# zengxianyu/sketchedit

Hardware: AMD Instinct MI355X
Metric: images/sec (higher is better)
Workload: dtype f32; 1 GPU; SketchEdit inference forward (netM+netG, use_cam, pool max) 256x256 batch 32 per GPU, procedural weights; global_batch=32, size=256, per_gpu_batch=32, execution=default, two streams

## Files before the change

sketchedit_amd/csrc/se_api.hip:

```cpp
#include "../../include/sketchedit_hip.h"
#include "../../include/sketchedit_png.h"
#include "../../include/sketchedit_jpg.h"
#include "../../include/sketchedit_jpg2.h"
#include "../../include/sketchedit_feather.h"
#include "../../include/sketchedit_fill.h"
#include "../../include/sketchedit_select.h"
#include "../../include/sketchedit_lasso.h"
#include "../../include/sketchedit_outline.h"
#include "se_kernels.h"
#include "se_pack.h"

#include <cstdarg>
#include <cstdint>
#include <cstdlib>
#include <cstdio>
#include <cstring>
#include <algorithm>
#include <map>
#include <mutex>
#include <numeric>
#include <string>
#include <vector>

using namespace se;
// ... 280 lines not shown
  p.src = src0; p.wpk = wimg; p.bias = L.d_b; p.dst = dst;
  p.B = B; p.Hin = Hin; p.Win = Win; p.C = C0; p.CG = CG; p.T = L.T; p.KW = KW;
  p.magicCG = (65536 + CG - 1) / CG; p.magicKW = 256 / KW + 1;
  for (int gi = 0; gi < nch * 8 + 8; ++gi)
    if (((gi * p.magicCG) >> 16) != gi / CG) return 0;
  for (int t = 0; t <= L.T + 8; ++t)
    if (((t * p.magicKW) >> 8) != t / KW) return 0;
  p.pad = pad; p.up2 = d.up ? 1 : 0; p.OH = Ho; p.OW = Wo;
  p.G = bf ? (L.G + 7) & ~7 : L.G;
  p.nch = nch; p.NP = L.NP;
  udiv_magic_host((unsigned)(C0 * es / 16), &p.div_cg_m, &p.div_cg_l);
  udiv_magic_host((unsigned)p.RW, &p.div_rw_m, &p.div_rw_l);
  p.ty = (Hin + TR - 1) / TR; p.tx = (Win + 15) / 16;
  p.act = d.act; p.bf16 = bf ? 1 : 0; p.xcd = xcd_remap_enabled();
  {
    const double alg = 2.0 * (double)B * Ho * Wo * d.cout * d.cin * d.k * d.k;
    const double exec = 2.0 * (double)B * Hin * Win * (d.up ? 4.0 : 1.0) * L.NP * (nch * (bf ? 64.0 : 32.0));
    set_launch_cost(alg, (double)es * ((double)B * Hin * Win * d.cin + (double)B * Ho * Wo * (d.cout / 2)), d.name, exec);
  }
  HIPCHK(c, launch_rtile(p, c->st));
  *done = true;
  return 0;
}

int run_gather(se_ctx* c, const Layer& L, bool bf, const float* src0, int C0, const float* src1, int C1, int src1_vec, float* dst,
               int B, int Hin, int Win, int Ho, int Wo, int pad) {
  const LayerDef& d = L.def;
  const DirectImage& di = L.direct[bf];
  const int es = bf ? 2 : 4, gran = bf ? 8 : 4;
  GConvParams p;
  memset(&p, 0, sizeof p);
  p.bf16 = bf ? 1 : 0;
  p.src0 = src0; p.src1 = src1 ? src1 : src0; p.wpk = di.w; p.bias = L.d_b; p.dst = dst; p.zeros = c->zeros;
  p.B = B; p.Hin = Hin; p.Win = Win; p.Ho = d.up ? Hin : Ho; p.Wo = d.up ? Win : Wo;
  p.up2 = d.up ? 1 : 0; p.OH = Ho; p.OW = Wo;
  p.C0 = C0; p.C1 = C1 ? C1 : C0; p.C0g = C0 / gran; p.CG = di.CG;
  const int KW = d.up ? 2 : d.k;
  p.T = L.T; p.KW = KW; p.stride = d.stride; p.dil = d.rate; p.pad = pad;
  p.magicCG = (65536 + di.CG - 1) / di.CG; p.magicKW = 256 / KW + 1; p.magicKH = L.T / KW;
  for (int gi = 0; gi < di.nch * 8 + 8; ++gi)
    if (((gi * p.magicCG) >> 16) != gi / di.CG) return fail(c, "layer %s: magic division check failed", d.name);
  for (int t = 0; t <= L.T + 8; ++t)
    if (((t * p.magicKW) >> 8) != t / KW) return fail(c, "layer %s: magic tap division check failed", d.name);
  const int Gs = bf ? (L.G + 7) & ~7 : L.G;
  if ((double)B * Hin * Win * (C0 > C1 ? C0 : C1) * es >= 2147483648.0 || (double)B * Ho * Wo * Gs * es >= 2147483648.0)
    return fail(c, "layer %s: a tensor of this launch exceeds 2^31 bytes (32-bit byte offsets) -- split the batch", d.name);
  for (int j = 0; j < p.magicKH; ++j) p.rep |= 1u << (j * KW);
  udiv_magic_host((unsigned)(p.Ho * p.Wo), &p.div_hw_m, &p.div_hw_l);
  udiv_magic_host((unsigned)p.Wo, &p.div_w_m, &p.div_w_l);
  p.Hlim = Hin; p.Wlim = Win;
  p.src1_vec = src1_vec; p.nch = di.nch; p.G = Gs; p.act = d.act; p.total_pix = B * p.Ho * p.Wo;
  p.xcd = xcd_remap_enabled();
  p.np_full = L.NP; p.nf_full = L.NP / 32; p.small_grid = c->low_latency ? 1 : 0;
  {
    const double alg = 2.0 * (double)B * Ho * Wo * d.cout * d.cin * d.k * d.k;
    const double exec = 2.0 * (double)B * p.Ho * p.Wo * (d.up ? 4.0 : 1.0) * L.NP * (di.nch * (bf ? 64.0 : 32.0));
    set_launch_cost(alg, (double)es * ((double)B * Hin * Win * d.cin + (double)B * Ho * Wo * (d.cout / 2)), d.name, exec);
  }
  HIPCHK(c, launch_gconv(L.cfg, p, c->st));
  return 0;
}

static bool rconv16_dual_ok(const Layer& L, const LayerDef& d, int Hin, int Win) {
  if (opt(OPT_RCONV16_DUAL) == 0) return false;
  return L.d_w16s && (d.rate % 2) == 0 && Win / d.rate == 8 && Hin / d.rate <= 8 && Hin / d.rate >= 4;
}

int run_gconv16(se_ctx* c, const Layer& L, const float* src0, int C0, const float* src1, int C1, int src1_vec, float* dst,
                int B, int Hin, int Win, int Ho, int Wo, int pad) {
  const LayerDef& d = L.def;
  if (!L.direct[1].w) return fail(c, "layer %s: no bf16 weight image", d.name);
  if ((C0 + C1) != L.direct[1].CG * 8) return fail(c, "layer %s: bf16 source channels %d+%d != packed %d", d.name, C0, C1, L.direct[1].CG * 8);
  const bool use_rconv = opt(OPT_RCONV16) != 0;
  {
    if (opt(OPT_VECBIAS) != 0 && use_rconv && !c->low_latency && src1 && src1_vec && c->vbias_ws && c->vec32 && L.d_w16s && L.d_wv16 &&
        d.k == 3 && d.stride == 1 && d.rate == 1 && !d.up && d.cin == 192 && d.cout == 192 && C0 == 96 && C1 == 96 &&
        Hin >= 12 && Win >= 12 && (long long)B * Hin * Win * 192 < (1ll << 31)) {
      HIPCHK(c, launch_vecbias(L.d_wv16, c->vec32, c->vbias_ws, B, 96, c->st, 1));
      RConvParams rp;
      memset(&rp, 0, sizeof rp);
      rp.src = src0; rp.wpk = L.d_w16s; rp.bias = L.d_b; rp.dst = dst; rp.vbias = c->vbias_ws;
      rp.B = B; rp.h = Hin; rp.w = Win; rp.d = 1; rp.hs = Hin; rp.ws = Win;
      rp.ty = (Hin + 7) / 8; rp.tx = (Win + 15) / 16;
      rp.act = d.act; rp.xcd = xcd_remap_enabled();
      const double alg = 2.0 * (double)B * Ho * Wo * d.cout * d.cin * 9;
      set_launch_cost(alg, 2.0 * 2.0 * (double)B * Hin * Win * 96, d.name, 2.0 * (double)B * Hin * Win * 192.0 * 864.0);
      HIPCHK(c, launch_rconv16(rp, c->st));
      return 0;
    }
  }
  if (use_rconv && !c->low_latency && d.k == 3 && d.stride == 1 && !d.up && d.cin == 96 && d.cout == 192 && !src1 && C0 == 96 &&
      (Hin % d.rate) == 0 && (Win % d.rate) == 0 && L.direct[1].nch == 14 && L.d_w16s && (long long)B * Hin * Win * 192 < (1ll << 31) &&
      ((Hin / d.rate >= 12 && Win / d.rate >= 12) || rconv16_dual_ok(L, d, Hin, Win))) {
    RConvParams rp;
    memset(&rp, 0, sizeof rp);
    rp.dual = !(Hin / d.rate >= 12 && Win / d.rate >= 12);
    rp.src = src0; rp.wpk = L.d_w16s; rp.bias = L.d_b; rp.dst = dst;
    rp.B = B; rp.h = Hin; rp.w = Win; rp.d = d.rate; rp.hs = Hin / d.rate; rp.ws = Win / d.rate;
    rp.ty = (rp.hs + 7) / 8; rp.tx = (rp.ws + 15) / 16;
    rp.act = d.act; rp.xcd = xcd_remap_enabled();
    const double alg = 2.0 * (double)B * Ho * Wo * d.cout * d.cin * 9;
    set_launch_cost(alg, 2.0 * 2.0 * (double)B * Hin * Win * 96, d.name, 2.0 * (double)B * Hin * Win * 192.0 * 864.0);
    HIPCHK(c, launch_rconv16(rp, c->st));
    return 0;
  }
  const bool use_rconv96 = opt(OPT_RCONV96) != 0;
// ... 2525 lines not shown
```

sketchedit_amd/csrc/se_attention.hip:

```cpp
#include "se_device.h"

#include <cstdlib>

namespace se {


template <bool BF16>
__global__ void att2_prep_kernel(const AttParams p) {
  const long idx = (long)blockIdx.x * 256 + threadIdx.x;
  const long nx = (long)p.B * p.h * p.w * (BF16 ? 12 : 24);
  if (idx < nx) {
    if (BF16) {
      const int cg = idx % 12;
      const long pix = idx / 12;
      const int b = pix / (p.h * p.w);
      const uint4 v = *(const uint4*)((const char*)p.x + idx * 16);
      const f32x4 r0 = *(const f32x4*)(p.rn + b * 96 + cg * 8), r1 = *(const f32x4*)(p.rn + b * 96 + cg * 8 + 4);
      *(uint4*)((char*)p.xn + idx * 16) =
          make_uint4(pack_bf16x2(bf16_lo(v.x) * r0[0], bf16_hi(v.x) * r0[1]), pack_bf16x2(bf16_lo(v.y) * r0[2], bf16_hi(v.y) * r0[3]),
                     pack_bf16x2(bf16_lo(v.z) * r1[0], bf16_hi(v.z) * r1[1]), pack_bf16x2(bf16_lo(v.w) * r1[2], bf16_hi(v.w) * r1[3]));
    } else {
      const int cg = idx % 24;
      const long pix = idx / 24;
      const int b = pix / (p.h * p.w);
// ... 98 lines not shown
#pragma unroll
    for (int o = 32; o > 0; o >>= 1) { a += __shfl_xor(a, o); bb += __shfl_xor(bb, o); g += __shfl_xor(g, o); }
    bb -= g;
  }
  if (lane == 0) { p.ea[gi] = a; p.eb[gi] = bb; }
}
__global__ __launch_bounds__(256) void att2_eoff4_kernel(const AttParams p) {
  const long gi = (long)blockIdx.x * 256 + threadIdx.x;
  if (gi >= (long)p.B * p.Rp) return;
  const int b = (int)(gi / p.Rp), k = (int)(gi - (long)b * p.Rp);
  const float* ea = p.ea + (size_t)b * p.Rp, *eb = p.eb + (size_t)b * p.Rp;
  auto at = [&](const float* t, int i) { return i < p.R ? t[i] : 0.f; };
  p.ea4[gi] = ((at(ea, k) + at(ea, k + 1)) + at(ea, k + p.wc)) + at(ea, k + p.wc + 1);
  const float b4 = ((at(eb, k) + at(eb, k + 1)) + at(eb, k + p.wc)) + at(eb, k + p.wc + 1);
  p.kadd2[gi] = fmaf(b4, p.kmul[gi], p.kadd[gi]);
}

template <int NT, int PT, bool BF16>
__global__ __launch_bounds__(256) void att2_pair_kernel(const AttParams p) {
  constexpr int PXB = BF16 ? 192 : 384;
  constexpr int PIX = PT * 64, NP = NT * 16;
  constexpr int XBYTES = PIX * 128, WBYTES = NP * 128;
  constexpr int NX = PT * 2, NW = (NT * 2 + 3) / 4;
  extern __shared__ __attribute__((aligned(16))) char smem[];
  char* Xb = smem;
  char* Wb = smem + 2 * XBYTES;

  const int tid = threadIdx.x, lane = tid & 63;
  const int w = __builtin_amdgcn_readfirstlane(tid >> 6);
  int b = blockIdx.z, bx = blockIdx.x, by = blockIdx.y;
  if (p.sym) {
    static_assert(PIX == 4 * NP, "tile enumeration");
    const int lb = xcd_tile(blockIdx.x, gridDim.x);
    b = lb / p.symT;
    const int t = lb - b * p.symT;
    int pn = (int)((sqrtf(64.f + 128.f * (float)t) - 8.f) * (1.f / 64.f));
    while (32 * (pn + 1) * (pn + 1) + 8 * (pn + 1) <= t) ++pn;
    while (32 * pn * pn + 8 * pn > t) --pn;
    const int u = t - (32 * pn * pn + 8 * pn);
    if (u < 64 * pn) {
      bx = u >> 4;
      by = 16 * pn + (u & 15);
    } else {
      const int v = u - 64 * pn;
      const int j = v < 16 ? 0 : (v < 28 ? 1 : (v < 36 ? 2 : 3));
      bx = 4 * pn + j;
      by = 16 * pn + 4 * j + (v - (j == 0 ? 0 : (j == 1 ? 16 : (j == 2 ? 28 : 36))));
    }
    if (by * NP >= p.R) return;
  }
  const int q0 = bx * PIX, k0 = by * NP;
  auto origin = [&](int i) -> unsigned {
    if (i >= p.R) return 0x80000000u;
    const int ry = i / p.wc, rx = i - ry * p.wc;
    return (unsigned)(((2 * ry) * p.w + 2 * rx) * PXB);
  };
  const se_i32x4 rs_q = make_rsrc((const char*)(p.sym ? p.xn : p.x) + (size_t)b * p.h * p.w * PXB, (unsigned)p.h * p.w * (unsigned)PXB);
  const se_i32x4 rs_k = make_rsrc((const char*)p.xn + (size_t)b * p.h * p.w * PXB, (unsigned)p.h * p.w * (unsigned)PXB);
  unsigned qo[NX], ko[NW];
#pragma unroll
  for (int i = 0; i < NX; ++i) qo[i] = origin(q0 + (i * 4 + w) * 8 + (lane >> 3));
#pragma unroll
  for (int j = 0; j < NW; ++j) ko[j] = (j * 4 + w) < NT * 2 ? origin(k0 + (j * 4 + w) * 8 + (lane >> 3)) : 0x80000000u;

  const int s_log = (lane & 7) ^ (4 * (w & 1) + (lane >> 4));
  int off0, off1;
  frag_offsets(lane, off0, off1);
  const unsigned lds_x = lds_addr_of(Xb), lds_w = lds_addr_of(Wb);

  auto stage = [&](int ch, int buf) {
    const int gi = ch * 8 + s_log;
    constexpr int GPP = BF16 ? 12 : 24;
    const int tap = (gi * (BF16 ? 5462 : 2731)) >> 16, cg = gi - tap * GPP;
    const unsigned doff = (unsigned)((__mul24(tap >> 1, p.w) + (tap & 1)) * PXB + cg * 16);
    const unsigned xdst = lds_x + buf * XBYTES, wdst = lds_w + buf * WBYTES;
#pragma unroll
    for (int i = 0; i < NX; ++i) bufdma16(qo[i] + doff, rs_q, xdst + (i * 4 + w) * 1024);
#pragma unroll
    for (int j = 0; j < NW; ++j) {
      const int rbk = j * 4 + w;
      if (rbk < NT * 2) bufdma16(ko[j] + doff, rs_k, wdst + rbk * 1024);
    }
  };

  f32x4 acc[NT][PT];
#pragma unroll
  for (int nt = 0; nt < NT; ++nt)
#pragma unroll
    for (int pt = 0; pt < PT; ++pt) acc[nt][pt] = (f32x4){0.f, 0.f, 0.f, 0.f};
  if (BF16 && p.e16) {
    const float* ea = p.ea + (size_t)b * p.Rp, *eb = p.eb + (size_t)b * p.Rp;
    float eq[PT];
#pragma unroll
    for (int pt = 0; pt < PT; ++pt) eq[pt] = ea[min(q0 + w * PT * 16 + pt * 16 + (lane & 15), p.Rp - 1)];
#pragma unroll
    for (int nt = 0; nt < NT; ++nt) {
      const f32x4 ek = *(const f32x4*)(eb + min(k0 + nt * 16 + (lane >> 4) * 4, p.Rp - 4));
#pragma unroll
      for (int pt = 0; pt < PT; ++pt) acc[nt][pt] = (f32x4){-(eq[pt] + ek[0]), -(eq[pt] + ek[1]), -(eq[pt] + ek[2]), -(eq[pt] + ek[3])};
    }
  }
  constexpr int NCH = BF16 ? 6 : 12;
  stage(0, 0);
  dma_wait_all();
  __syncthreads();
  for (int ch = 0; ch < NCH; ++ch) {
    const int buf = ch & 1;
    if (ch + 1 < NCH) stage(ch + 1, buf ^ 1);
    if (BF16) mfma_chunk16<NT, PT>(acc, Wb + buf * WBYTES, Xb + buf * XBYTES + w * PT * 2048, off0, off1);
    else mfma_chunk<NT, PT>(acc, Wb + buf * WBYTES, Xb + buf * XBYTES + w * PT * 2048, off0, off1);
    dma_wait_all();
    __syncthreads();
  }
  constexpr int TS = NT * 16 + 4;
  static_assert(4 * PT * 16 * TS * 4 <= 2 * XBYTES + 2 * WBYTES, "transpose buffer exceeds the staging buffers");
  float* T = (float*)smem + w * (PT * 16 * TS);
  const int q = lane >> 4;
#pragma unroll
  for (int nt = 0; nt < NT; ++nt)
#pragma unroll
    for (int pt = 0; pt < PT; ++pt) *(f32x4*)(T + (pt * 16 + (lane & 15)) * TS + nt * 16 + q * 4) = acc[nt][pt];
  constexpr int PPR = NT * 4;
  constexpr int RPI = 64 / PPR;
  const int pc = lane % PPR, pr = lane / PPR;
  const int j = k0 + pc * 4;
#pragma unroll
  for (int rr = 0; rr < PT * 16; rr += RPI) {
    const int row = rr + pr;
    const f32x4 v = *(const f32x4*)(T + row * TS + pc * 4);
    const int i = q0 + w * PT * 16 + row;
    if (i < p.R && j < p.Rp) {
      if (BF16 && p.e16) {
        typedef _Float16 h4 __attribute__((ext_vector_type(4)));
        typedef unsigned u32x2 __attribute__((ext_vector_type(2)));
        auto sat = [](float t) { return __builtin_amdgcn_fmed3f(t, -65504.f, 65504.f); };
        const h4 hv = (h4){(_Float16)sat(v[0]), (_Float16)sat(v[1]), (_Float16)sat(v[2]), (_Float16)sat(v[3])};
        __builtin_nontemporal_store(__builtin_bit_cast(u32x2, hv), (u32x2*)((char*)p.E + (((size_t)b * p.R + i) * p.Rp + j) * 2));
      } else __builtin_nontemporal_store(v, (f32x4*)(p.E + ((size_t)b * p.R + i) * p.Rp + j));
    }
  }
  if (!BF16 && p.sym && k0 >= q0 + PIX) {
    constexpr int PPM = PT * 4;
    constexpr int RPM = 64 / PPM;
    const int mc = lane % PPM, mr = lane / PPM;
    const int qcol = q0 + w * PT * 16 + mc * 4;
#pragma unroll
    for (int kk0 = 0; kk0 < NT * 16; kk0 += RPM) {
      const int kk = kk0 + mr;
      const float* t = T + (mc * 4) * TS + kk;
      const f32x4 v = (f32x4){t[0], t[TS], t[2 * TS], t[3 * TS]};
      const int srow = k0 + kk;
      if (srow < p.R && qcol < p.Rp) __builtin_nontemporal_store(v, (f32x4*)(p.E + ((size_t)b * p.R + srow) * p.Rp + qcol));
    }
  }
}

DEVFN bool tile_order(long q, int B, int ny, int nx, int& b, int& y, int& x) {
  const int ty = (ny + 7) >> 3, tx = (nx + 7) >> 3;
  const long per = (long)ty * tx * 64;
  b = (int)(q / per);
  const int rem = (int)(q - (long)b * per), t = rem >> 6, in = rem & 63;
  y = (t / tx) * 8 + (in >> 3);
  x = (t % tx) * 8 + (in & 7);
  return b < B && y < ny && x < nx;
}
static inline long tile_order_count(int B, int ny, int nx) { return (long)B * ((ny + 7) >> 3) * ((nx + 7) >> 3) * 64; }

template <bool BF16>
__global__ __launch_bounds__(256) void att2_softmax_kernel(const AttParams p) {
  const int lane = threadIdx.x & 63;
  int b, iy, ix;
  if (!tile_order((long)xcd_tile(blockIdx.x, gridDim.x) * 4 + (threadIdx.x >> 6), p.B, p.hs, p.ws, b, iy, ix)) return;
  const int r0 = iy * p.wc + ix;
  const float* E0 = p.E + ((size_t)b * p.R + r0) * p.Rp;
  const float* E1 = E0 + p.Rp;
  const float* E2 = E0 + (size_t)p.wc * p.Rp;
  const float* E3 = E2 + p.Rp;
  const float* vr = p.validR + (size_t)b * p.Rp;
  float* P = p.P + ((size_t)b * p.R + r0) * p.Rp;
  unsigned short* P16 = (unsigned short*)p.P + ((size_t)b * p.R + r0) * p.Rp;
  const int o2 = p.wc, o3 = p.wc + 1;
  auto score = [&](int s, float v) { return (E0[s] + E1[s + 1] + E2[s + o2] + E3[s + o3]) * v * p.scale; };
  float m = -INFINITY;
  for (int s = lane; s < p.R; s += 64) {
    const float v = vr[s];
    if (v >= 0.f) {
      const float sc = score(s, v);
      if (!BF16) P[s] = sc;
      m = fmaxf(m, sc);
    }
  }
#pragma unroll
  for (int o = 32; o > 0; o >>= 1) m = fmaxf(m, __shfl_xor(m, o));
  float sum = 0.f;
  for (int s = lane; s < p.R; s += 64) {
    const float v = vr[s];
    if (v >= 0.f) {
      const float e = expf((BF16 ? score(s, v) : P[s]) - m);
      if (!BF16) P[s] = e;
      sum += e;
    }
  }
#pragma unroll
// ... 662 lines not shown
#pragma unroll
  for (int pt = 0; pt < PT; ++pt) {
    const int i = t0 + (w * PT + pt) * 16 + (lane & 15);
    if (i >= p.R) continue;
    const int yy = i / p.wc, xx = i - yy * p.wc;
    char* o = (char*)p.out + (((long)(b * p.h + 2 * yy + py) * p.w + 2 * xx + px) * 96 + rh * NP) * ES;
#pragma unroll
    for (int nt = 0; nt < NT; ++nt) {
      const f32x4 a = acc[nt][pt];
      if (BF16) *(uint2*)(o + (nt * 16 + q * 4) * 2) = make_uint2(pack_bf16x2(a[0], a[1]), pack_bf16x2(a[2], a[3]));
      else *(f32x4*)(o + (nt * 16 + q * 4) * 4) = a;
    }
  }
}

template <bool BF16>
__global__ void att2_similar_kernel(const AttParams p) {
  const long idx = (long)blockIdx.x * 256 + threadIdx.x;
  if (idx >= (long)p.B * p.L * p.L) return;
  const int i = idx % p.L;
  const long bj = idx / p.L;
  const int j = bj % p.L, b = bj / p.L;
  const int r = (i / p.ws) * p.wc + i % p.ws, s = (j / p.ws) * p.wc + j % p.ws;
  const size_t at = ((size_t)b * p.R + r) * p.Rp + s;
  p.similar[idx] = BF16 ? bf16_lo(((const unsigned short*)p.P)[at]) : p.P[at];
}

static bool att_lds_form(int wc) {
  return wc % 4 == 0 && wc <= 124 && opt(OPT_ATT_PTILDE_LDS) != 0;
}
static bool att_fused(bool bf16, int Rp, int wc) {
  const int e1 = opt(OPT_ATT_FUSED), e2 = opt(OPT_ATT_FUSED_BF16);
  const int f32mode = e1 < 0 ? -1 : (e1 != 0 ? 1 : 0);
  if (bf16) {
    if (e2 == 0) return false;
    if (e2 > 0) return f32mode < 0 ? att_lds_form(wc) : f32mode == 1;
    return f32mode != 0 && att_lds_form(wc);
  }
  return f32mode < 0 ? (Rp <= 1024 || att_lds_form(wc)) : f32mode == 1;
}

template <bool BF16>
static void enqueue_att2_prep(const AttParams& p, hipStream_t st) {
  const long n = (long)p.B * p.h * p.w * (BF16 ? 12 : 24);
  hipLaunchKernelGGL(att2_prep_kernel<BF16>, dim3((unsigned)((n + 255) / 256)), dim3(256), 0, st, p);
  hipLaunchKernelGGL(att2_transpose_kernel<BF16>, dim3(p.Rp / 32, 4, p.B), dim3(256), 0, st, p);
}

template <bool BF16>
static hipError_t launch_attention_v2_t(const AttParams& p0, hipStream_t st) {
  AttParams p = p0;
  const bool fused = att_fused(BF16, p.Rp, p.wc) && !p.similar && p.stats;
  p.Pt = fused ? p.P : p.E;
  p.sym = (!BF16 && opt(OPT_ATT_SYM) != 0) ? 1 : 0;
  const bool stats_lds = opt(OPT_ATT_STATS_LDS) != 0;
  p.e16 = (BF16 && fused && att_lds_form(p.wc) && stats_lds && opt(OPT_ATT_E16) != 0) ? 1 : 0;
  {
    const long n = (long)p.B * p.h * p.w * (BF16 ? 12 : 24);
    if (p.guard < p.wc + 8 || ((n + 255) / 256) * 256 < (long)p.guard) return hipErrorInvalidValue;
    ProfScope ps_(st, PL_ATT_PREP);
    enqueue_att2_prep<BF16>(p, st);
    if (p.e16) {
      const long nr = (long)p.B * p.Rp;
      hipLaunchKernelGGL(att2_emean1_kernel<BF16>, dim3(p.hc, p.B), dim3(384), 0, st, p);
      hipLaunchKernelGGL(att2_emean2_kernel, dim3(p.B), dim3(384), 0, st, p);
      hipLaunchKernelGGL(att2_eoff_kernel<BF16>, dim3((unsigned)((nr + 3) / 4)), dim3(256), 0, st, p);
      hipLaunchKernelGGL(att2_eoff4_kernel, dim3((unsigned)((nr + 255) / 256)), dim3(256), 0, st, p);
    }
  }
  {
    const double alg_flops = 2.0 * p.B * (double)p.L * p.L * 1536.0;
    const double alg_bytes = (BF16 ? 2.0 : 4.0) * 2.0 * p.B * (double)p.h * p.w * 96;
    const long big_grid = (long)((p.R + 255) / 256) * ((p.R + 63) / 64) * p.B;
    if (big_grid >= 512) {
      constexpr int NT = 4, PT = 4;
      constexpr int LDS = 2 * PT * 64 * 128 + 2 * NT * 16 * 128;
      hipError_t e = ensure_max_lds((const void*)att2_pair_kernel<NT, PT, BF16>, LDS);
      if (e != hipSuccess) return e;
      dim3 grid((p.R + PT * 64 - 1) / (PT * 64), (p.Rp + NT * 16 - 1) / (NT * 16), p.B);
      if (p.sym) {
        const int np = ((int)grid.y + 15) / 16;
        p.symT = 32 * np * np + 8 * np;
        grid = dim3((unsigned)(p.symT * p.B));
      }
      set_launch_cost(alg_flops, alg_bytes, nullptr, 2.0 * (double)grid.x * grid.y * grid.z * (PT * 64.0) * (NT * 16.0) * 384.0);
      set_launch_grid((long)grid.x * grid.y * grid.z);
      ProfScope ps_(st, PL_ATT_SCORE, p.sym ? "att_pair_sym" : "att_pair_all");
      hipLaunchKernelGGL((att2_pair_kernel<NT, PT, BF16>), grid, dim3(256), LDS, st, p);
    } else {
      constexpr int NT = 2, PT = 2;
      constexpr int LDS = 2 * PT * 64 * 128 + 2 * NT * 16 * 128;
      hipError_t e = ensure_max_lds((const void*)att2_pair_kernel<NT, PT, BF16>, LDS);
      if (e != hipSuccess) return e;
      dim3 grid((p.R + PT * 64 - 1) / (PT * 64), (p.Rp + NT * 16 - 1) / (NT * 16), p.B);
      if (p.sym) {
        const int np = ((int)grid.y + 15) / 16;
        p.symT = 32 * np * np + 8 * np;
        grid = dim3((unsigned)(p.symT * p.B));
      }
      set_launch_cost(alg_flops, alg_bytes, nullptr, 2.0 * (double)grid.x * grid.y * grid.z * (PT * 64.0) * (NT * 16.0) * 384.0);
      set_launch_grid((long)grid.x * grid.y * grid.z);
      ProfScope ps_(st, PL_ATT_SCORE, p.sym ? "att_pair_sym" : "att_pair_all");
      hipLaunchKernelGGL((att2_pair_kernel<NT, PT, BF16>), grid, dim3(256), LDS, st, p);
    }
  }
  if (fused) {
// ... 109 lines not shown
```

sketchedit_amd/csrc/se_device.h:

```cpp
#pragma once
#include "se_kernels.h"

namespace se {

typedef float f32x4 __attribute__((ext_vector_type(4)));
typedef float f32x2 __attribute__((ext_vector_type(2)));
#define DEVFN __device__ __forceinline__

DEVFN void glds16(const void* gsrc, unsigned lds_addr) {
  unsigned keep;
  asm volatile(
      "s_mov_b32 %0, m0\n\t"
      "s_mov_b32 m0, %2\n\t"
      "s_nop 0\n\t"
      "global_load_lds_dwordx4 %1, off\n\t"
      "s_mov_b32 m0, %0"
      : "=&s"(keep)
      : "v"(gsrc), "s"(lds_addr)
      : "memory");
}
DEVFN void glds16_s(const void* sbase, unsigned voff, unsigned lds_addr) {
  unsigned keep;
  asm volatile(
      "s_mov_b32 %0, m0\n\t"
// ... 33 lines not shown
      "s_mov_b32 m0, %3\n\t"
      "s_nop 0\n\t"
      "buffer_load_dword %1, %2, 0 offen lds\n\t"
      "s_mov_b32 m0, %0"
      : "=&s"(keep)
      : "v"(voff), "s"(rsrc), "s"(lds_addr)
      : "memory");
}
DEVFN void dma_wait_all() { asm volatile("s_waitcnt vmcnt(0)" ::: "memory"); }

DEVFN unsigned lds_addr_of(const void* p) {
  return (unsigned)(size_t)(const __attribute__((address_space(3))) char*)p;
}

DEVFN float sigmoidf_(float x) { return 1.f / (1.f + expf(-x)); }
DEVFN float fast_exp(float x) { return __expf(x); }
DEVFN float fast_rcp(float x) { return __builtin_amdgcn_rcpf(x); }
DEVFN float elu_fast(float x) {
  const float e = __builtin_amdgcn_exp2f(fminf(x, 0.f) * 1.44269504088896340736f) - 1.f;
  return x > 0.f ? x : e;
}
DEVFN float sigmoid_fast(float x) { return fast_rcp(1.f + fast_exp(-x)); }
DEVFN float act_fast(float x, float eluw) {
  const float n = __builtin_amdgcn_fmed3f(x * 1.44269504088896340736f, -__builtin_inff(), 0.f);
  const float neg = fmaf(__builtin_amdgcn_exp2f(n), eluw, -eluw);
  return __builtin_amdgcn_fmed3f(x, neg, __builtin_inff());
}
DEVFN float tanh_fast(float x) { return 1.f - 2.f * fast_rcp(1.f + fast_exp(2.f * x)); }

DEVFN unsigned udiv_magic(unsigned x, unsigned m, int l) {
  const unsigned t = __umulhi(m, x);
  return (t + ((x - t) >> (l < 1 ? l : 1))) >> (l > 1 ? l - 1 : 0);
}

DEVFN int xcd_tile(int bid, int nblocks) {
  const int q = nblocks >> 3, r = nblocks & 7;
  const int xcd = bid & 7, idx = bid >> 3;
  return (xcd < r ? xcd * (q + 1) : r * (q + 1) + (xcd - r) * q) + idx;
}

DEVFN bool class_tile(int bid, int ntiles, int xcd_remap, int& tile, int& cls) {
  const int xcd = bid & 7, g = bid >> 3;
  cls = g & 3;
  const int b2 = ((g >> 2) << 3) | xcd;
  if (b2 >= ntiles) return false;
  tile = xcd_remap ? xcd_tile(b2, ntiles) : b2;
  return true;
}
static inline int class_tile_grid(int ntiles) { return 4 * ((ntiles + 7) & ~7); }

struct NoHook { DEVFN void operator()(int) const {} };
template <int NT, int PT, typename Hook = NoHook>
DEVFN void mfma_chunk(f32x4 (&acc)[NT][PT], const char* __restrict__ Wt, const char* __restrict__ Xt, int off0,
                      int off1, Hook hook = Hook()) {
  f32x4 xb[2][PT];
#pragma unroll
  for (int half = 0; half < 2; ++half)
#pragma unroll
    for (int pt = 0; pt < PT; ++pt) xb[half][pt] = *(const f32x4*)(Xt + pt * 2048 + (half ? off1 : off0));
  f32x4 wn = *(const f32x4*)(Wt + off0);
#pragma unroll
  for (int half = 0; half < 2; ++half) {
#pragma unroll
    for (int nt = 0; nt < NT; ++nt) {
      const f32x4 wa = wn;
      if (nt + 1 < NT) wn = *(const f32x4*)(Wt + (nt + 1) * 2048 + (half ? off1 : off0));
      else if (half == 0) wn = *(const f32x4*)(Wt + off1);
#pragma unroll
      for (int r = 0; r < 4; ++r) {
#pragma unroll
        for (int pt = 0; pt < PT; ++pt)
          acc[nt][pt] = __builtin_amdgcn_mfma_f32_16x16x4f32(wa[r], xb[half][pt][r], acc[nt][pt], 0, 0, 0);
      }
      hook(half * NT + nt);
    }
  }
}

typedef __bf16 bf16x8 __attribute__((ext_vector_type(8)));
DEVFN unsigned pack_bf16x2(float lo, float hi) {
  unsigned r;
  asm("v_cvt_pk_bf16_f32 %0, %1, %2" : "=v"(r) : "v"(lo), "v"(hi));
  return r;
}
DEVFN float bf16_lo(unsigned u) { return __uint_as_float(u << 16); }
DEVFN float bf16_hi(unsigned u) { return __uint_as_float(u & 0xffff0000u); }

template <int NT, int PT, typename Hook = NoHook>
DEVFN void mfma_chunk16(f32x4 (&acc)[NT][PT], const char* __restrict__ Wt, const char* __restrict__ Xt, int off0,
                        int off1, Hook hook = Hook()) {
  constexpr int NU = 2 * NT, DEPTH = NU < 6 ? NU : 6;
  bf16x8 xb[2][PT];
#pragma unroll
  for (int half = 0; half < 2; ++half)
#pragma unroll
    for (int pt = 0; pt < PT; ++pt) xb[half][pt] = *(const bf16x8*)(Xt + pt * 2048 + (half ? off1 : off0));
  bf16x8 wq[DEPTH];
#pragma unroll
  for (int u = 0; u < DEPTH; ++u) wq[u] = *(const bf16x8*)(Wt + (u % NT) * 2048 + (u / NT ? off1 : off0));
  __builtin_amdgcn_sched_barrier(0);
#pragma unroll
  for (int u = 0; u < NU; ++u) {
    const int half = u / NT, nt = u % NT;
    const bf16x8 wa = wq[u % DEPTH];
    if (u + DEPTH < NU) wq[u % DEPTH] = *(const bf16x8*)(Wt + ((u + DEPTH) % NT) * 2048 + ((u + DEPTH) / NT ? off1 : off0));
    __builtin_amdgcn_sched_barrier(0);
#pragma unroll
    for (int pt = 0; pt < PT; ++pt)
      acc[nt][pt] = __builtin_amdgcn_mfma_f32_16x16x32_bf16(wa, xb[half][pt], acc[nt][pt], 0, 0, 0);
    hook(u);
    __builtin_amdgcn_sched_barrier(0);
  }
}

DEVFN void frag_offsets(int lane, int& off0, int& off1) {
  const int swz = (lane >> 1) & 7;
  off0 = (lane & 15) * 128 + (((lane >> 4) ^ swz) << 4);
  off1 = (lane & 15) * 128 + (((4 + (lane >> 4)) ^ swz) << 4);
}

DEVFN unsigned load_dword_within(const unsigned char* p, const unsigned char* lo, const unsigned char* hi) {
  if (p >= lo && p + 4 <= hi) return *(const unsigned*)p;
  unsigned v = 0;
#pragma unroll
  for (int i = 0; i < 4; ++i)
    if (p + i >= lo && p + i < hi) v |= (unsigned)p[i] << (8 * i);
  return v;
}
DEVFN unsigned load4_within(const unsigned char* a, const unsigned char* lo, const unsigned char* hi) {
  const unsigned char* a0 = (const unsigned char*)((size_t)a & ~(size_t)3);
  const int sh = (int)((size_t)a & 3) * 8;
  const unsigned d0 = load_dword_within(a0, lo, hi);
  if (!sh) return d0;
  return (d0 >> sh) | (load_dword_within(a0 + 4, lo, hi) << (32 - sh));
}
DEVFN unsigned clear_locked(unsigned sel, unsigned lk) {
#pragma unroll
  for (int p = 0; p < 4; ++p)
    if ((lk >> (8 * p)) & 255u) sel &= ~(255u << (8 * p));
  return sel;
}

struct ProfScope {
  hipStream_t st;
  int idx = -1;
  ProfScope(hipStream_t s, int label, const char* form = nullptr);
  ~ProfScope();
};

}
```

sketchedit_amd/csrc/se_gconv.hip:

```cpp
#include "se_device.h"

#include <cstdlib>

namespace se {

template <int NT, int PT, bool MIXED, int WPS, bool FAST, bool SPLIT, bool BF16>
__global__ __launch_bounds__(256, WPS) void gconv_kernel(const GConvParams p) {
  constexpr int PIX = PT * 64;
  constexpr int NP = NT * 16;
  constexpr int ES = BF16 ? 2 : 4;
  constexpr int XBYTES = PIX * 128, WBYTES = NP * 128;
  constexpr int NX = PT * 2;
  extern __shared__ __attribute__((aligned(16))) char smem[];
  char* Xb = smem;
  char* Wb = smem + 2 * XBYTES;
  int2* rowtab = (int2*)smem;

  const int tid = threadIdx.x, lane = tid & 63;
  const float eluw = p.act == 0 ? 1.f : 0.f;
  const int w = __builtin_amdgcn_readfirstlane(tid >> 6);
  int tile_idx = p.xcd ? xcd_tile(blockIdx.x, gridDim.x) : (int)blockIdx.x, cls = 0;
  if (p.up2 && !class_tile((int)blockIdx.x, (p.total_pix + PIX - 1) / PIX, p.xcd, tile_idx, cls)) return;
  const int tile_base = tile_idx * PIX;
  const int py = cls >> 1, px = cls & 1;
// ... 82 lines not shown
    fast_head(ch);
#pragma unroll
    for (int q = 0; q < NPIECE; ++q) fast_piece(ch, buf, q);
  };
  auto stage_any = [&](int ch, int buf) {
    const int gi = ch * 8 + s_log;
    const int tap = (gi * p.magicCG) >> 16, cg = gi - tap * p.CG;
    const int ky = (tap * p.magicKW) >> 8, kx = tap - ky * p.KW;
    const int dy = ky * p.dil - pady, dx = kx * p.dil - padx;
    const bool tapok = tap < p.T;
    const bool first = cg < p.C0g;
    const char* base = (const char*)(first ? p.src0 : p.src1);
    const int cs = (first ? p.C0 : p.C1) * ES;
    const int coff = (first ? cg : cg - p.C0g) * 16;
    const bool vec = (!first) && p.src1_vec;
    const unsigned xdst = lds_x + buf * XBYTES;
#pragma unroll
    for (int i = 0; i < NX; ++i) {
      int iy = (ryx[i] >> 16) + dy, ix = (ryx[i] & 0xffff) + dx;
      const bool ok = tapok & ((unsigned)iy < (unsigned)p.Hlim) & ((unsigned)ix < (unsigned)p.Wlim);
      iy >>= p.ushift;
      ix >>= p.ushift;
      const unsigned pix = vec ? (unsigned)rb[i] : (unsigned)((rb[i] * p.Hin + iy) * p.Win + ix);
      const char* g = base + (size_t)pix * (unsigned)cs + (unsigned)coff;
      g = ok ? g : (const char*)p.zeros;
      glds16(g, xdst + (i * 4 + w) * 1024);
    }
    const unsigned wdst = lds_w + buf * WBYTES;
    const float* wsrc = wbase + (size_t)ch * npf * 32 + lane * 4;
#pragma unroll
    for (int j = 0; j < (NT * 2 + 3) / 4; ++j) {
      const int rbk = j * 4 + w;
      if (rbk < NT * 2) glds16(wsrc + full_rbk(rbk) * 256, wdst + rbk * 1024);
    }
  };
  auto stage = [&](int ch, int buf) {
    if (FAST) stage_fast(ch, buf);
    else stage_any(ch, buf);
  };

  f32x4 acc[NT][PT];
#pragma unroll
  for (int nt = 0; nt < NT; ++nt)
#pragma unroll
    for (int pt = 0; pt < PT; ++pt) acc[nt][pt] = (f32x4){0.f, 0.f, 0.f, 0.f};

  stage(0, 0);
  dma_wait_all();
  __syncthreads();
  for (int ch = 0; ch < p.nch; ++ch) {
    const int buf = ch & 1;
    if (FAST) {
      const bool more = ch + 1 < p.nch;
      if (more) fast_head(ch + 1);
      constexpr int SLOTS = NT, PER = (NPIECE + SLOTS - 1) / SLOTS;
      auto hook = [&](int slot) {
        if (more) {
#pragma unroll
          for (int u = 0; u < PER; ++u) fast_piece(ch + 1, buf ^ 1, slot * PER + u);
        }
      };
      if (BF16) mfma_chunk16<NT, PT>(acc, Wb + buf * WBYTES, Xb + buf * XBYTES + w * PT * 2048, off0, off1, hook);
      else mfma_chunk<NT, PT>(acc, Wb + buf * WBYTES, Xb + buf * XBYTES + w * PT * 2048, off0, off1, hook);
    } else {
      if (ch + 1 < p.nch) stage(ch + 1, buf ^ 1);
      if (BF16) mfma_chunk16<NT, PT>(acc, Wb + buf * WBYTES, Xb + buf * XBYTES + w * PT * 2048, off0, off1);
      else mfma_chunk<NT, PT>(acc, Wb + buf * WBYTES, Xb + buf * XBYTES + w * PT * 2048, off0, off1);
    }
    dma_wait_all();
    __syncthreads();
  }

  const int q = lane >> 4;
  auto out_off = [&](int pidx) -> size_t {
    if (!p.up2) return (size_t)pidx * p.G;
    const int b = (int)udiv_magic((unsigned)pidx, p.div_hw_m, p.div_hw_l), rem = pidx - b * HoWo;
    const int yy = (int)udiv_magic((unsigned)rem, p.div_w_m, p.div_w_l), xx = rem - yy * p.Wo;
    return ((size_t)(b * p.OH + 2 * yy + py) * p.OW + 2 * xx + px) * p.G;
  };
  if (!MIXED) {
    constexpr int NF = NT / 2;
    const int nff = SPLIT ? p.nf_full : NF;
#pragma unroll
    for (int nt = 0; nt < NF; ++nt) {
      const int c0 = (grp * NF + nt) * 16 + q * 4;
      const f32x4 bf = *(const f32x4*)(p.bias + c0);
      const f32x4 bg = *(const f32x4*)(p.bias + nff * 16 + c0);
#pragma unroll
      for (int pt = 0; pt < PT; ++pt) {
        const int pidx = tile_base + (w * PT + pt) * 16 + (lane & 15);
        f32x4 o;
#pragma unroll
        for (int r = 0; r < 4; ++r) {
          const float f = acc[nt][pt][r] + bf[r];
          const float g = acc[nt + NF][pt][r] + bg[r];
          const float a = act_fast(f, eluw);
          o[r] = a * sigmoid_fast(g);
        }
        if (c0 < p.G && pidx < p.total_pix) {
          if (BF16) *(uint2*)((char*)p.dst + (out_off(pidx) + c0) * 2) = make_uint2(pack_bf16x2(o[0], o[1]), pack_bf16x2(o[2], o[3]));
          else *(f32x4*)(p.dst + out_off(pidx) + c0) = o;
        }
      }
    }
  } else {
#pragma unroll
    for (int nt = 0; nt < NT; ++nt) {
      const int c0 = (grp * NT + nt) * 8 + (q & 1) * 4 + (q >> 1) * 2;
      const f32x4 bq = *(const f32x4*)(p.bias + (grp * NT + nt) * 16 + q * 4);
#pragma unroll
      for (int pt = 0; pt < PT; ++pt) {
        const int pidx = tile_base + (w * PT + pt) * 16 + (lane & 15);
        const f32x4 v = acc[nt][pt] + bq;
        const auto s02 = __builtin_amdgcn_permlane32_swap(__float_as_uint(v[0]), __float_as_uint(v[2]), false, false);
        const auto s13 = __builtin_amdgcn_permlane32_swap(__float_as_uint(v[1]), __float_as_uint(v[3]), false, false);
        const float f0 = __uint_as_float(s02[0]), g0 = __uint_as_float(s02[1]);
        const float f1 = __uint_as_float(s13[0]), g1 = __uint_as_float(s13[1]);
        float2 o;
        o.x = act_fast(f0, eluw) * sigmoid_fast(g0);
        o.y = act_fast(f1, eluw) * sigmoid_fast(g1);
// ... 72 lines not shown
```

sketchedit_amd/csrc/se_kernels.h:

```cpp
#pragma once
#include <hip/hip_runtime.h>
#include <stddef.h>
#include <stdint.h>

#include <vector>

struct se_window;

namespace se {

enum ProfLabel { PL_GCONV_N192 = 0, PL_GCONV_N96, PL_GCONV_N48, PL_GCONV_N24, PL_WINO_N192, PL_WINO_N96, PL_WINO_UP96, PL_SMALL_CONV, PL_PACK, PL_COLREDUCE,
                 PL_ATT_PREP, PL_ATT_SCORE, PL_ATT_SOFTMAX, PL_ATT_BOXSUM, PL_ATT_PV, PL_LAYOUT,
                 PL_ATT_STREAM_STATS, PL_ATT_STREAM_OUT, PL_RESIZE_H, PL_RESIZE_V, PL_WINDOW_GATHER, PL_WINDOW_BORDER, PL_WINDOW_PASTE,
                 PL_WINDOW_RESAMPLE_H, PL_WINDOW_PASTE_V, PL_WINDOW_SAVE, PL_WINDOW_SWAP, PL_WINDOW_LOCK_GATHER, PL_WINDOW_PASTE_LOCKED,
                 PL_WINDOW_PASTE_V_LOCKED, PL_SKETCH_TILES, PL_SKETCH_STROKES, PL_PNG_ROWS, PL_PNG_STRIPES,
                 PL_PNG_FINISH, PL_JPG_BLOCKS, PL_JPG_ROWS, PL_JPG_FINISH, PL_JPG2_BLOCKS, PL_JPG2_HIST, PL_JPG2_TABLES,
                 PL_WINDOW_PASTE_FEATHER, PL_FILL_MASKS, PL_FILL_KEEP, PL_SELECT_SIMILAR, PL_SELECT_FLOOD, PL_SELECT_GROW,
                 PL_LASSO_FILL, PL_PLANE_COMBINE, PL_OUTLINE_COUNT, PL_OUTLINE_SCAN, PL_OUTLINE_EMIT, PL_COUNT };
const char* prof_label_name(int l);
struct Profiler {
  struct Rec { int label; const char* name; const char* form; double flops; double exec_flops; double bytes; long blocks; hipEvent_t a, b; };
  std::vector<Rec> recs;
  std::vector<hipEvent_t> pool;
  size_t used = 0;
// ... 12 lines not shown
  X(RTILE_DENSE, 1)                                          \
  X(RTILE_D5W, 1)                                        \
  X(TEST_OFFSET_LIMIT, 0)  \
  X(TEST_POISON, 0)       \
  X(RCONV16, 1) X(RCONV16_DUAL, 1) X(RCONV96, 1) X(VECBIAS, 1)                                                  \
  X(WINOGRAD, 1) X(WINOGRAD48, 1) X(WINOGRAD_UP, 1) X(WINOGRAD_UP48, 1)                                         \
  X(WINOGRAD_F43, 1)      \
  X(GCONV_FAST, 1) X(FORK_DEFAULT, 1) X(LL_WINO_MIN_WG, 64) X(LL_WINO48_MIN_WG, 128)                            \
  X(ATT_FUSED, -1) X(ATT_FUSED_BF16, -1) X(ATT_PTILDE_LDS, 1) X(ATT_STATS_LDS, 1) X(ATT_E16, 1) X(ATT_SYM, 1)   \
  X(ATT_STREAM, 0)
enum Opt {
#define X(name, dflt) OPT_##name,
  SE_OPTIONS(X)
#undef X
  OPT_COUNT
};
int opt(int o);
int opt_set(const char* name, int value);
int opt_get(const char* name, int* value);
void opt_reset();
long long opt_epoch();

struct GConvParams {
  const float* src0;
  const float* src1;
  const float* wpk;
  const float* bias;
  float* dst;
  const float* zeros;
  int B, Hin, Win, Ho, Wo;
  int C0, C1;
  int C0g, CG;
  int T, KW;
  int magicCG, magicKW;
  int magicKH;
  unsigned rep;
  unsigned div_hw_m, div_w_m;
  int div_hw_l, div_w_l;
  int stride, dil, pad;
  int ushift;
  int up2;
  int OH, OW;
  int Hlim, Wlim;
  int src1_vec;
  int nch;
  int G;
  int act;
  int total_pix;
  int xcd;
  int np_full;
  int nf_full;
  int bf16;
  int small_grid;
};

static inline void udiv_magic_host(unsigned d, unsigned* m, int* l) {
  int ll = 0;
  while ((1ull << ll) < d) ++ll;
  *l = ll;
  *m = (unsigned)(((1ull << 32) * ((1ull << ll) - d)) / d + 1);
}

enum GConvCfg { GC_N192 = 0, GC_N96 = 1, GC_N48 = 2, GC_N24 = 3 };
static inline int gconv_np(int cfg) { return cfg == GC_N192 ? 192 : cfg == GC_N96 ? 96 : cfg == GC_N48 ? 48 : 32; }
static inline bool gconv_mixed(int cfg) { return cfg >= GC_N48; }

hipError_t launch_gconv(int cfg, const GConvParams& p, hipStream_t st);

struct WinoParams {
  const float* src;
  const float* src1;
  int src1_vec;
  const float* upk;
  const float* bias;
  float* dst;
  int B, h, w, d;
  int th, tw;
  int total_tiles;
  int act;
  int xcd;
  unsigned div_tpi_m, div_tw_m, div_d_m;
  int div_tpi_l, div_tw_l, div_d_l;
  const float* vbias;
};
hipError_t launch_wino(const WinoParams& p, hipStream_t st);
hipError_t launch_vecbias(const float* wv, const float* vec, float* T, int B, int C1, hipStream_t st, int round_vec = 0);
hipError_t launch_wino24(const WinoParams& p, hipStream_t st);
hipError_t launch_wino24_c48(const WinoParams& p, hipStream_t st);
hipError_t launch_wino48(const WinoParams& p, hipStream_t st);
hipError_t launch_wino48_c24(const WinoParams& p, hipStream_t st);
hipError_t launch_winoup(const WinoParams& p, hipStream_t st);
hipError_t launch_winoup48(const WinoParams& p, hipStream_t st);

struct RConvParams {
  const void* src;
  const void* wpk;
  const float* bias;
  void* dst;
  int B, h, w, d;
  int hs, ws;
  int ty, tx;
  int act;
  int xcd;
  const float* vbias;
  int dual;
};
// ... 65 lines not shown
hipError_t launch_small_conv(const SmallConvParams& p, hipStream_t st);

hipError_t launch_pack_m(const float* image, const float* sketch, float* dst4, int B, int H, int W, hipStream_t st);
hipError_t launch_pack_g(const float* x, const float* x2, const float* mask, const float* mask2, const float* guide,
                         float* coarse8, float* style8, int B, int H, int W, int no_mask_cc, int joint,
                         hipStream_t st);
hipError_t launch_nchw_to_nhwc(const float* src, float* dst, int B, int C, int Cpad, int H, int W, hipStream_t st);
hipError_t launch_dequantize_u8(const unsigned char* rgb, const unsigned char* sk8, const float* lut, float* image, float* sketch,
                                int B, int H, int W, hipStream_t st);
hipError_t launch_nhwc_to_nchw(const float* src, float* dst, int B, int C, int Cstride, int H, int W, hipStream_t st);
hipError_t launch_quantize_u8(const float* composed, const float* mask, unsigned char* rgb, unsigned char* m8, int B, int H,
                              int W, hipStream_t st);
hipError_t launch_colreduce(const float* x, float* partial, float* out, int B, int HW, int C, int op, hipStream_t st,
                            int x_bf16 = 0, float* out_bf16 = nullptr);
hipError_t launch_pack_m16(const float* image, const float* sketch, float* dst8, int B, int H, int W, hipStream_t st);
hipError_t launch_pack_g16(const float* x, const float* x2, const float* mask, const float* mask2, const float* guide,
                           float* coarse8, float* style8, int B, int H, int W, int no_mask_cc, int joint, hipStream_t st);
hipError_t launch_nchw_to_nhwc16(const float* src, float* dst, int B, int C, int Cpad, int H, int W, hipStream_t st);
hipError_t launch_nhwc16_to_nchw(const float* src, float* dst, int B, int C, int Cstride, int H, int W, hipStream_t st);
static const int COLREDUCE_SPLITS = 128;

struct AttParams {
  const float* x;
  const float* rn;
  float* xn;
  const float* hard;
  float* valid;
  float* S;
  float* out;
  int B, h, w, hs, ws, L, Lp;
  float scale;
  float th;
  int hc, wc, R, Rp;
  float* xT;
  float* E;
  float* P;
  float* Pt;
  float* stats;
  float* kmul;
  float* kadd;
  int guard;
  float* validR;
  float* similar;
  int bf16;
  int e16;
  float* emean;
  float* epart;
  float* ea;
  float* eb;
  float* ea4;
  float* kadd2;
  int sym;
  int symT;
};
hipError_t launch_attention(const AttParams& p, hipStream_t st);
hipError_t launch_att2_prep(const AttParams& p, hipStream_t st);
hipError_t launch_attention_stream(const AttParams& p, hipStream_t st);
int att_stream_xt_tail();

int resample_ksize(int in, int out, int filter);
int resample_coeffs(int in, int out, int filter, int* bounds, int* kk);
enum { RESIZE_OUT_U8 = 0, RESIZE_OUT_IMAGE_F32 = 1, RESIZE_OUT_SKETCH_F32 = 2, RESIZE_OUT_LOCK_U8 = 3 };
struct ResizeOut {
  int mode;
  unsigned char* u8;
  float* f32;
  const float* lut;
  int H, W;
};
hipError_t launch_resample_h(const unsigned char* in, const int* d_bounds, const int* d_kk, const int* h_bounds, int ksize,
                             int B, int Hrows, int Win, int Wout, int C, const ResizeOut& o, hipStream_t st);
hipError_t launch_resample_v(const unsigned char* in, const int* d_bounds, const int* d_kk, int ksize, int B, int Hin, int Hout,
                             int W, int C, const ResizeOut& o, hipStream_t st);
hipError_t launch_window_resample_h(const se_window* d_wins, const int* d_bounds, const int* d_kk, const int* h_bounds, int ksize,
                                    int B, int hs, int ws, int Wout, int C, const ResizeOut& o, hipStream_t st);
hipError_t launch_window_paste_v(const se_window* d_wins, const unsigned char* rgb, const unsigned char* m8, const int* d_bounds,
                                 const int* d_kk, int ksize, int B, int Hin, int hs, int P, int ws, hipStream_t st, bool locked = false);
hipError_t launch_window_lock_resample_h(const se_window* d_wins, const int* d_bounds, const int* d_kk, const int* h_bounds, int ksize,
                                         int B, int hs, int ws, int Wout, const ResizeOut& o, hipStream_t st);
constexpr int RESAMPLE_MAX_KSIZE = 8191;

hipError_t launch_window_gather(const se_window* d_wins, const float* lut, float* image, float* sketch, int B, int H, int W,
                                hipStream_t st);
hipError_t launch_window_border(const se_window* d_wins, const unsigned char* m8, int* hits, int B, int H, int W, int hs, int ws,
                                hipStream_t st);
hipError_t launch_window_paste(const se_window* d_wins, const unsigned char* rgb, const unsigned char* m8, int B, int H, int W,
                               hipStream_t st, bool locked = false);
hipError_t launch_window_paste_feather(const se_window* d_wins, const unsigned char* rgb, const unsigned char* m8, int B, int hs, int ws,
                                       int radius, hipStream_t st);
hipError_t launch_window_lock_gather(const se_window* d_wins, unsigned char* out, int B, int H, int W, hipStream_t st);
hipError_t launch_window_journal(const se_window* d_wins, int B, int hs, int ws, bool swap, hipStream_t st);
hipError_t launch_sketch_tiles(const unsigned char* plane, int Hi, int Wi, int tile, int* tiles_out, hipStream_t st);
hipError_t launch_sketch_strokes(const se_window* d_wins, int B, int hs, int ws, const int* segs, long nseg_sum, unsigned char* sketch_out,
                                 hipStream_t st);
hipError_t launch_fill_masks(const unsigned char* fill, const unsigned char* lock, float* hole, float* hard, float* zero, int B, int H,
                             int W, hipStream_t st);
hipError_t launch_fill_keep(const se_window* d_wins, int B, int hs, int ws, hipStream_t st);
hipError_t launch_select_similar(const unsigned char* frame, int Hi, int Wi, int seed_y, int seed_x, int tolerance, int contiguous,
                                 unsigned char* state, hipStream_t st);
hipError_t launch_select_flood(unsigned char* state, int Hi, int Wi, unsigned* changed, hipStream_t st);
hipError_t launch_select_grow(const unsigned char* state, int Hi, int Wi, int grow, unsigned char* out, hipStream_t st);
hipError_t launch_lasso_fill(const int* edges, int N, int Hi, int Wi, unsigned char* plane_out, hipStream_t st);
hipError_t launch_plane_combine(const unsigned char* a, const unsigned char* b, int Hi, int Wi, int op, unsigned char* out, hipStream_t st);
hipError_t launch_outline_count(const unsigned char* plane, int Hi, int Wi, int* cnt, hipStream_t st);
hipError_t launch_outline_scan(int* cnt, int Hi, int Wi, int cap, int* info_out, hipStream_t st);
hipError_t launch_outline_emit(const unsigned char* plane, int Hi, int Wi, const int* offs, int* edges_out, int cap, hipStream_t st);
// ... 23 lines not shown
```

Measured before the change: 2964 images/sec.

## Skip padded half-chunk MFMAs in gconv and swizzle attention transpose LDS

The grouped conv now skips the second-half MFMA pass on the last K chunk whenever the host determines that the remaining taps times channel groups fit in the first half, so no work is spent on zero padding. The attention score kernel swaps its padded LDS transpose buffer for an XOR-swizzled layout in the f32 NT=4/PT=4 case, which removes the padding and is meant to avoid bank conflicts on both the row and the symmetric column readback. It also replaces an integer division by wc with a magic-number multiply. The skip condition relies on the padded half being all zeros; if it is not, results are wrong.

New measurement: 2971 images/sec (median of 6 runs). No clear change (+0.2%).

```diff
diff --git a/sketchedit_amd/csrc/se_api.hip b/sketchedit_amd/csrc/se_api.hip
--- a/sketchedit_amd/csrc/se_api.hip
+++ b/sketchedit_amd/csrc/se_api.hip
@@ -356,6 +356,7 @@
   p.src1_vec = src1_vec; p.nch = di.nch; p.G = Gs; p.act = d.act; p.total_pix = B * p.Ho * p.Wo;
   p.xcd = xcd_remap_enabled();
   p.np_full = L.NP; p.nf_full = L.NP / 32; p.small_grid = c->low_latency ? 1 : 0;
+  p.skip_half = L.T * di.CG <= (di.nch - 1) * 8 + 4 ? 1 : 0;
   {
     const double alg = 2.0 * (double)B * Ho * Wo * d.cout * d.cin * d.k * d.k;
     const double exec = 2.0 * (double)B * p.Ho * p.Wo * (d.up ? 4.0 : 1.0) * L.NP * (di.nch * (bf ? 64.0 : 32.0));
diff --git a/sketchedit_amd/csrc/se_attention.hip b/sketchedit_amd/csrc/se_attention.hip
--- a/sketchedit_amd/csrc/se_attention.hip
+++ b/sketchedit_amd/csrc/se_attention.hip
@@ -174,7 +174,7 @@
   const int q0 = bx * PIX, k0 = by * NP;
   auto origin = [&](int i) -> unsigned {
     if (i >= p.R) return 0x80000000u;
-    const int ry = i / p.wc, rx = i - ry * p.wc;
+    const int ry = (int)udiv_magic((unsigned)i, p.div_wc_m, p.div_wc_l), rx = i - ry * p.wc;
     return (unsigned)(((2 * ry) * p.w + 2 * rx) * PXB);
   };
   const se_i32x4 rs_q = make_rsrc((const char*)(p.sym ? p.xn : p.x) + (size_t)b * p.h * p.w * PXB, (unsigned)p.h * p.w * (unsigned)PXB);
@@ -234,14 +234,19 @@
     dma_wait_all();
     __syncthreads();
   }
-  constexpr int TS = NT * 16 + 4;
+  constexpr bool SWZ = !BF16 && NT == 4 && PT == 4;
+  constexpr int TS = SWZ ? NT * 16 : NT * 16 + 4;
   static_assert(4 * PT * 16 * TS * 4 <= 2 * XBYTES + 2 * WBYTES, "transpose buffer exceeds the staging buffers");
   float* T = (float*)smem + w * (PT * 16 * TS);
+  auto swz = [](int row) -> int { return SWZ ? ((row ^ (row >> 2)) & 7) << 2 : 0; };
   const int q = lane >> 4;
 #pragma unroll
   for (int nt = 0; nt < NT; ++nt)
 #pragma unroll
-    for (int pt = 0; pt < PT; ++pt) *(f32x4*)(T + (pt * 16 + (lane & 15)) * TS + nt * 16 + q * 4) = acc[nt][pt];
+    for (int pt = 0; pt < PT; ++pt) {
+      const int row = pt * 16 + (lane & 15);
+      *(f32x4*)(T + row * TS + ((nt * 16 + q * 4) ^ swz(row))) = acc[nt][pt];
+    }
   constexpr int PPR = NT * 4;
   constexpr int RPI = 64 / PPR;
   const int pc = lane % PPR, pr = lane / PPR;
@@ -249,7 +254,7 @@
 #pragma unroll
   for (int rr = 0; rr < PT * 16; rr += RPI) {
     const int row = rr + pr;
-    const f32x4 v = *(const f32x4*)(T + row * TS + pc * 4);
+    const f32x4 v = *(const f32x4*)(T + row * TS + ((pc * 4) ^ swz(row)));
     const int i = q0 + w * PT * 16 + row;
     if (i < p.R && j < p.Rp) {
       if (BF16 && p.e16) {
@@ -264,13 +269,14 @@
   if (!BF16 && p.sym && k0 >= q0 + PIX) {
     constexpr int PPM = PT * 4;
     constexpr int RPM = 64 / PPM;
-    const int mc = lane % PPM, mr = lane / PPM;
+    const int mc = SWZ ? (lane & 7) + 8 * (lane >> 5) : lane % PPM, mr = SWZ ? (lane >> 3) & 3 : lane / PPM;
     const int qcol = q0 + w * PT * 16 + mc * 4;
 #pragma unroll
     for (int kk0 = 0; kk0 < NT * 16; kk0 += RPM) {
       const int kk = kk0 + mr;
-      const float* t = T + (mc * 4) * TS + kk;
-      const f32x4 v = (f32x4){t[0], t[TS], t[2 * TS], t[3 * TS]};
+      const float* t = T + (mc * 4) * TS;
+      const f32x4 v = (f32x4){t[kk ^ swz(mc * 4)], t[TS + (kk ^ swz(mc * 4 + 1))], t[2 * TS + (kk ^ swz(mc * 4 + 2))],
+                              t[3 * TS + (kk ^ swz(mc * 4 + 3))]};
       const int srow = k0 + kk;
       if (srow < p.R && qcol < p.Rp) __builtin_nontemporal_store(v, (f32x4*)(p.E + ((size_t)b * p.R + srow) * p.Rp + qcol));
     }
@@ -1039,6 +1045,7 @@
   AttParams p = p0;
   const bool fused = att_fused(BF16, p.Rp, p.wc) && !p.similar && p.stats;
   p.Pt = fused ? p.P : p.E;
+  udiv_magic_host((unsigned)p.wc, &p.div_wc_m, &p.div_wc_l);
   p.sym = (!BF16 && opt(OPT_ATT_SYM) != 0) ? 1 : 0;
   const bool stats_lds = opt(OPT_ATT_STATS_LDS) != 0;
   p.e16 = (BF16 && fused && att_lds_form(p.wc) && stats_lds && opt(OPT_ATT_E16) != 0) ? 1 : 0;
diff --git a/sketchedit_amd/csrc/se_device.h b/sketchedit_amd/csrc/se_device.h
--- a/sketchedit_amd/csrc/se_device.h
+++ b/sketchedit_amd/csrc/se_device.h
@@ -109,7 +109,7 @@
 struct NoHook { DEVFN void operator()(int) const {} };
 template <int NT, int PT, typename Hook = NoHook>
 DEVFN void mfma_chunk(f32x4 (&acc)[NT][PT], const char* __restrict__ Wt, const char* __restrict__ Xt, int off0,
-                      int off1, Hook hook = Hook()) {
+                      int off1, bool skip1 = false, Hook hook = Hook()) {
   f32x4 xb[2][PT];
 #pragma unroll
   for (int half = 0; half < 2; ++half)
@@ -118,18 +118,20 @@
   f32x4 wn = *(const f32x4*)(Wt + off0);
 #pragma unroll
   for (int half = 0; half < 2; ++half) {
-#pragma unroll
-    for (int nt = 0; nt < NT; ++nt) {
-      const f32x4 wa = wn;
-      if (nt + 1 < NT) wn = *(const f32x4*)(Wt + (nt + 1) * 2048 + (half ? off1 : off0));
-      else if (half == 0) wn = *(const f32x4*)(Wt + off1);
-#pragma unroll
-      for (int r = 0; r < 4; ++r) {
-#pragma unroll
-        for (int pt = 0; pt < PT; ++pt)
-          acc[nt][pt] = __builtin_amdgcn_mfma_f32_16x16x4f32(wa[r], xb[half][pt][r], acc[nt][pt], 0, 0, 0);
+    if (half == 0 || !skip1) {
+#pragma unroll
+      for (int nt = 0; nt < NT; ++nt) {
+        const f32x4 wa = wn;
+        if (nt + 1 < NT) wn = *(const f32x4*)(Wt + (nt + 1) * 2048 + (half ? off1 : off0));
+        else if (half == 0) wn = *(const f32x4*)(Wt + off1);
+#pragma unroll
+        for (int r = 0; r < 4; ++r) {
+#pragma unroll
+          for (int pt = 0; pt < PT; ++pt)
+            acc[nt][pt] = __builtin_amdgcn_mfma_f32_16x16x4f32(wa[r], xb[half][pt][r], acc[nt][pt], 0, 0, 0);
+        }
+        hook(half * NT + nt);
       }
-      hook(half * NT + nt);
     }
   }
 }
@@ -145,7 +147,7 @@
 
 template <int NT, int PT, typename Hook = NoHook>
 DEVFN void mfma_chunk16(f32x4 (&acc)[NT][PT], const char* __restrict__ Wt, const char* __restrict__ Xt, int off0,
-                        int off1, Hook hook = Hook()) {
+                        int off1, bool skip1 = false, Hook hook = Hook()) {
   constexpr int NU = 2 * NT, DEPTH = NU < 6 ? NU : 6;
   bf16x8 xb[2][PT];
 #pragma unroll
@@ -156,8 +158,7 @@
 #pragma unroll
   for (int u = 0; u < DEPTH; ++u) wq[u] = *(const bf16x8*)(Wt + (u % NT) * 2048 + (u / NT ? off1 : off0));
   __builtin_amdgcn_sched_barrier(0);
-#pragma unroll
-  for (int u = 0; u < NU; ++u) {
+  auto step = [&](int u) {
     const int half = u / NT, nt = u % NT;
     const bf16x8 wa = wq[u % DEPTH];
     if (u + DEPTH < NU) wq[u % DEPTH] = *(const bf16x8*)(Wt + ((u + DEPTH) % NT) * 2048 + ((u + DEPTH) / NT ? off1 : off0));
@@ -167,6 +168,12 @@
       acc[nt][pt] = __builtin_amdgcn_mfma_f32_16x16x32_bf16(wa, xb[half][pt], acc[nt][pt], 0, 0, 0);
     hook(u);
     __builtin_amdgcn_sched_barrier(0);
+  };
+#pragma unroll
+  for (int u = 0; u < NT; ++u) step(u);
+  if (!skip1) {
+#pragma unroll
+    for (int u = NT; u < NU; ++u) step(u);
   }
 }
 
diff --git a/sketchedit_amd/csrc/se_gconv.hip b/sketchedit_amd/csrc/se_gconv.hip
--- a/sketchedit_amd/csrc/se_gconv.hip
+++ b/sketchedit_amd/csrc/se_gconv.hip
@@ -158,6 +158,7 @@
     const int buf = ch & 1;
     if (FAST) {
       const bool more = ch + 1 < p.nch;
+      const bool skip1 = !more && p.skip_half;
       if (more) fast_head(ch + 1);
       constexpr int SLOTS = NT, PER = (NPIECE + SLOTS - 1) / SLOTS;
       auto hook = [&](int slot) {
@@ -166,12 +167,13 @@
           for (int u = 0; u < PER; ++u) fast_piece(ch + 1, buf ^ 1, slot * PER + u);
         }
       };
-      if (BF16) mfma_chunk16<NT, PT>(acc, Wb + buf * WBYTES, Xb + buf * XBYTES + w * PT * 2048, off0, off1, hook);
-      else mfma_chunk<NT, PT>(acc, Wb + buf * WBYTES, Xb + buf * XBYTES + w * PT * 2048, off0, off1, hook);
+      if (BF16) mfma_chunk16<NT, PT>(acc, Wb + buf * WBYTES, Xb + buf * XBYTES + w * PT * 2048, off0, off1, skip1, hook);
+      else mfma_chunk<NT, PT>(acc, Wb + buf * WBYTES, Xb + buf * XBYTES + w * PT * 2048, off0, off1, skip1, hook);
     } else {
+      const bool skip1 = ch + 1 == p.nch && p.skip_half;
       if (ch + 1 < p.nch) stage(ch + 1, buf ^ 1);
-      if (BF16) mfma_chunk16<NT, PT>(acc, Wb + buf * WBYTES, Xb + buf * XBYTES + w * PT * 2048, off0, off1);
-      else mfma_chunk<NT, PT>(acc, Wb + buf * WBYTES, Xb + buf * XBYTES + w * PT * 2048, off0, off1);
+      if (BF16) mfma_chunk16<NT, PT>(acc, Wb + buf * WBYTES, Xb + buf * XBYTES + w * PT * 2048, off0, off1, skip1);
+      else mfma_chunk<NT, PT>(acc, Wb + buf * WBYTES, Xb + buf * XBYTES + w * PT * 2048, off0, off1, skip1);
     }
     dma_wait_all();
     __syncthreads();
diff --git a/sketchedit_amd/csrc/se_kernels.h b/sketchedit_amd/csrc/se_kernels.h
--- a/sketchedit_amd/csrc/se_kernels.h
+++ b/sketchedit_amd/csrc/se_kernels.h
@@ -88,6 +88,7 @@
   int nf_full;
   int bf16;
   int small_grid;
+  int skip_half;
 };
 
 static inline void udiv_magic_host(unsigned d, unsigned* m, int* l) {
@@ -259,6 +260,8 @@
   float* kadd2;
   int sym;
   int symT;
+  unsigned div_wc_m;
+  int div_wc_l;
 };
 hipError_t launch_attention(const AttParams& p, hipStream_t st);
 hipError_t launch_att2_prep(const AttParams& p, hipStream_t st);
```
